# microsoft/Sora

Measured on AMD Instinct MI355X. Metric: IQ Msamples/s through 802.11a 54 Mbps RX PHY, higher is better.
Workload: dtype int16 IQ / u8 path metrics

## Files before the change

### sora_amd/build.py

```python
import os
import shutil
import subprocess
import sys
from concurrent.futures import ThreadPoolExecutor

HERE = os.path.dirname(os.path.abspath(__file__))
CSRC = os.path.join(HERE, "csrc")
OBJ = os.path.join(HERE, "lib", "obj")
LIB = os.path.join(HERE, "lib", "libsora_hip.so")
SOURCES = ["k_scan.hip", "k_rx.hip", "k_vit16.hip", "k_vitwin.hip", "k_stage.hip", "k_tx.hip", "k_tx11n.hip", "k_tx_ht40.hip", "k_tx11b.hip", "k_rx11b.hip", "k_11n.hip", "k_rx11n.hip",
    "k_ht40.hip", "k_deliver.hip", "sora_hip.cpp", "sora_shard.cpp"]
HEADERS = ["dev_arith.h", "dev_viterbi.h", "dev_vit16.h", "dev_winplan.h", "dev_vitwin.h", "dev_11n.h", "dev_ht40.h", "dev_pilot11a.h", "dev_sym11a.h", "rx_types.h", "kernels.h", "host_calls.h",
           "host_trellis.h", os.path.join("..", "..", "include", "sora_hip.h")]
FLAGS = ["--offload-arch=gfx950", "-O3", "-std=c++17", "-fPIC", "-fvisibility=hidden", "-x", "hip"]


def hipcc():
    for c in (os.environ.get("HIPCC"), shutil.which("hipcc"), "/opt/rocm/bin/hipcc"):
        if c and os.path.exists(c):
            return c
    raise RuntimeError("hipcc not found: libsora_hip.so cannot be built (there is no CPU fallback)")


def _newest_header():
    return max(os.path.getmtime(os.path.join(CSRC, h)) for h in HEADERS)


def _obj(src):
    return os.path.join(OBJ, os.path.splitext(src)[0] + ".o")


def _stale(src, hdr_t):
    o = _obj(src)
    return not os.path.exists(o) or os.path.getmtime(o) < max(os.path.getmtime(os.path.join(CSRC, src)), hdr_t)


def needs_build():
    if not os.path.exists(LIB):
        return True
    t = os.path.getmtime(LIB)
    return any(os.path.getmtime(os.path.join(CSRC, f)) > t for f in SOURCES + HEADERS)


INFO = os.path.join(HERE, "lib", "libsora_hip.buildinfo.json")


def sources_sha256():
    import hashlib
    h = hashlib.sha256()
    for f in sorted(SOURCES) + sorted(HEADERS):
        with open(os.path.join(CSRC, f), "rb") as fh:
            h.update(f.encode()); h.update(fh.read())
    return h.hexdigest()


def build_info():
    import json, socket, hashlib
    out = {"library": os.path.relpath(LIB, os.path.dirname(HERE)), "exists": os.path.exists(LIB)}
    if out["exists"]:
        with open(LIB, "rb") as fh:
            out["library_sha256"] = hashlib.sha256(fh.read()).hexdigest()
    try:
        with open(INFO) as fh:
            st = json.load(fh)
    except Exception:
        st = None
    now = sources_sha256()
    out["stamp"] = st
    out["sources_sha256_now"] = now
    out["built_from_this_tree"] = bool(st) and st.get("sources_sha256") == now and st.get("library_sha256") == out.get("library_sha256")
    out["built_on_this_host"] = bool(st) and st.get("host") == socket.gethostname()
    return out


def _write_info(ncompiled):
    import json, socket, hashlib, time
    try:
        ver = subprocess.run([hipcc(), "--version"], capture_output=True, text=True).stdout.splitlines()[0]
    except Exception:
        ver = None
    with open(LIB, "rb") as fh:
        lib_sha = hashlib.sha256(fh.read()).hexdigest()
    with open(INFO, "w") as fh:
        json.dump({"sources_sha256": sources_sha256(), "library_sha256": lib_sha, "host": socket.gethostname(), "built_at_unix": int(time.time()), "hipcc": ver,
                   "flags": FLAGS, "objects_compiled_in_this_build": ncompiled}, fh, indent=1)


def build_variant(name, defines):
    out_dir = os.path.join(HERE, "lib", "variants"); os.makedirs(out_dir, exist_ok=True)
    out = os.path.join(out_dir, name + ".so")
    if any(d.startswith(("SORA_DBG_", "SORA_SCAN_PROBE")) for d in defines) and "SORA_TOOLS" not in defines:
        defines = list(defines) + ["SORA_TOOLS"]
    cmd = [hipcc()] + FLAGS + ["-shared", "-w"] + ["-D" + d for d in defines] + [os.path.join(CSRC, f) for f in SOURCES] + ["-ldl", "-o", out]
    subprocess.check_call(cmd)
    return out

# ... 30 lines not shown
```

### sora_amd/csrc/k_rx.hip

```cpp
#include <hip/hip_runtime.h>
#include <utility>
#include "kernels.h"
#include "dev_sym11a.h"
#include "dev_viterbi.h"
#include "dev_winplan.h"
#include "dev_vitwin.h"

namespace sora {

struct FrameLds {
    uint32_t eq[4][4][64];
    uint8_t  soft[4][4][288];
    uint8_t  demap[1024];
    int4     trk[4][4];
    int      nsym_of[4];
    short    st0[4][4];
};
template <bool SHARED>
__device__ __forceinline__ void frame_symbols(const RxArgs& A, uint32_t j, FrameLds& lds, bool valid = true)
{
    uint32_t (&s_eq)[4][4][64] = lds.eq; uint8_t (&s_soft)[4][4][288] = lds.soft; const uint8_t* s_demap = lds.demap;
    const int w = threadIdx.x >> 6, lane = threadIdx.x & 63, g = lane >> 4, e = lane & 15;
    const Tables& T = A.T;
    const uint32_t f = valid ? A.joblist[j] : 0u;
// ... 784 lines not shown
        if (w < nwords) {
            const uint32_t sb = phase == 255 ? 0u : lds.seq4[(phase + 32u * w) % 127u];
            const uint32_t o = __builtin_amdgcn_alignbyte(hi[k], lo[k], 2u) ^ sb;
            s_buf[w] = o;
            mp32[w] = o;
            if (hp32) hp32[w] = o;
        }
    }
    __builtin_amdgcn_fence(__ATOMIC_RELEASE, "wavefront");
    __builtin_amdgcn_wave_barrier();
    __builtin_amdgcn_fence(__ATOMIC_ACQUIRE, "wavefront");
    const int n = L >= 4 ? (int)L - 4 : 0;
    uint32_t crc;
    if (n >= 4) {
        crc = crc32_wave(bytes, n, s_crc, s_z, lane);
    } else {
        crc = 0xFFFFFFFFu;
        for (int i = 0; i < n; i++) crc = (crc >> 8) ^ s_crc[(bytes[i] ^ crc) & 0xFF];
    }
    if (lane == 0) {
        uint32_t fcs = 0;
        if (L >= 4) fcs = (uint32_t)bytes[L - 4] | ((uint32_t)bytes[L - 3] << 8) | ((uint32_t)bytes[L - 2] << 16) | ((uint32_t)bytes[L - 1] << 24);
        r.crc32 = fcs;
        r.error_code = ((~crc) == fcs) ? E_FRAME_OK : E_CRC32_FAIL;
    }
}

__global__ void __launch_bounds__(256) k_finish(RxArgs A)
{
    __shared__ FinishLds L;
    finish_tables_to_lds(A, L);
    __syncthreads();
    const JobRef jr = locate_job(blockIdx.x * 4 + (threadIdx.x >> 6), A.njobs);
    if (!jr.ok) return;
    finish_frame(A, A.joblist[jr.list * A.nrows + jr.idx], L);
}

struct PipeFallbackGate {
    WinProofGate proof; const RxArgs* A; FrameLds* lds; bool gave_up;
    __device__ __forceinline__ bool operator()(uint32_t list, uint32_t fa, uint32_t fb, bool hasB) const
    {
        if (!gave_up) return proof(list, fa, fb, hasB);
        frame_symbols<false>(*A, list * A->nrows + fa, *lds);
        if (hasB) frame_symbols<false>(*A, list * A->nrows + fb, *lds);
        __builtin_amdgcn_fence(__ATOMIC_RELEASE, "agent"); __builtin_amdgcn_fence(__ATOMIC_ACQUIRE, "agent");
        return true;
    }
};
template <bool PIPE>
__device__ __forceinline__ void win_redo_finish_body(const VitJob* jobs, const uint32_t* hdr, uint32_t jstride, uint32_t target, uint32_t vstride,
                                                     const uint16_t* vecs, const uint8_t* soft, uint8_t* out, unsigned long long* stats, const RxArgs& A, uint32_t* host_note)
{
    __shared__ FinishLds L;
    finish_tables_to_lds(A, L);
    auto after = [&](uint32_t list, uint32_t fa, uint32_t fb, bool hasB) {
        finish_frame(A, A.joblist[list * A.nrows + fa], L);
        if (hasB) finish_frame(A, A.joblist[list * A.nrows + fb], L);
    };
    const WinProofGate proof{ jobs, hdr, jstride, target, vstride, vecs, stats };
    if constexpr (PIPE) {
        __shared__ FrameLds F;
        reinterpret_cast<uint32_t*>(F.demap)[threadIdx.x] = reinterpret_cast<const uint32_t*>(A.T.demap)[threadIdx.x];
        __syncthreads();
        const bool gave_up = __builtin_amdgcn_readfirstlane((int)A.pipe_flags[0]) != 0;
        if (gave_up && blockIdx.x == 0 && threadIdx.x == 0) {
            if (stats) atomicAdd(&stats[4u * kWinStatBanks], 1ull);
            if (host_note) __hip_atomic_store(host_note, 1u, __ATOMIC_RELAXED, __HIP_MEMORY_SCOPE_SYSTEM);
        }
        viterbi_kernel_body<256, 24, 3>(jobs, hdr, 0u, jstride, soft, out, PipeFallbackGate{ proof, &A, &F, gave_up }, after);
    } else {
        __syncthreads();
        viterbi_kernel_body<256, 24, 3>(jobs, hdr, 0u, jstride, soft, out, proof, after);
    }
}
__global__ void __launch_bounds__(256) k_win_redo_finish(const VitJob* jobs, const uint32_t* hdr, uint32_t jstride, uint32_t target, uint32_t vstride,
                                                         const uint16_t* vecs, const uint8_t* soft, uint8_t* out, unsigned long long* stats, RxArgs A)
{ win_redo_finish_body<false>(jobs, hdr, jstride, target, vstride, vecs, soft, out, stats, A, nullptr); }
__global__ void __launch_bounds__(256) k_win_redo_finish_pipe(const VitJob* jobs, const uint32_t* hdr, uint32_t jstride, uint32_t target, uint32_t vstride,
                                                              const uint16_t* vecs, const uint8_t* soft, uint8_t* out, unsigned long long* stats, RxArgs A, uint32_t* host_note)
{ win_redo_finish_body<true>(jobs, hdr, jstride, target, vstride, vecs, soft, out, stats, A, host_note); }

struct PackedRow { uint32_t capture_id, start_sample, end_sample, error_code, rate_kbps; uint16_t length, nsym; uint32_t crc32; int16_t cfo_est;
    uint16_t flags; uint32_t mpdu_offset; };
__global__ void __launch_bounds__(1024) k_pack(const FrameRow* frames, const uint32_t* nframes, const CapDesc* caps, uint32_t ncaps, uint32_t max_frames,
                                               PackedRow* rows, uint32_t* nrows_out)
{
    __shared__ uint32_t s_scan[1024];
    __shared__ uint32_t s_base;
    const uint32_t t = threadIdx.x;
    if (t == 0) s_base = 0;
    __syncthreads();
    for (uint32_t c0 = 0; c0 < ncaps; c0 += 1024) {
        const uint32_t c = c0 + t;
        const uint32_t found = c < ncaps ? nframes[c] : 0u;
        const uint32_t n = min(found, max_frames);
        s_scan[t] = n;
        __syncthreads();
        for (uint32_t o = 1; o < 1024; o <<= 1) {
            const uint32_t v = t >= o ? s_scan[t - o] : 0u;
            __syncthreads();
            s_scan[t] += v;
            __syncthreads();
        }
        const uint32_t first = s_base + s_scan[t] - n;
        for (uint32_t i = 0; i < n; i++) {
            const FrameRow& r = frames[(size_t)c * max_frames + i];
            PackedRow o;
            o.capture_id = caps[c].capture_id; o.start_sample = r.start_sample; o.end_sample = r.end_sample; o.error_code = r.error_code;
            o.rate_kbps = r.rate_kbps; o.length = r.length; o.nsym = r.nsym; o.crc32 = r.crc32; o.cfo_est = r.cfo_est;
            o.flags = (i + 1 == n && found > max_frames) ? 1u : 0u;
            o.mpdu_offset = r.slot0 * (uint32_t)kOutPerSlot;
            rows[first + i] = o;
        }
        __syncthreads();
        if (t == 1023) s_base += s_scan[1023];
        __syncthreads();
    }
    if (t == 0) *nrows_out = s_base;
}


__global__ void __launch_bounds__(256) k_soft_pack3(const uint8_t* soft8, const uint32_t* off8, const uint32_t* nsoft, const uint16_t* flen, const uint32_t* out_off,
                                                    int code_rate, uint8_t* packed, VitJob* jobs)
{
    const uint32_t j = blockIdx.x, mine = nsoft[j], at = (off8[j] + 1u) / 2u;
    const uint8_t* in = soft8 + off8[j];
    for (uint32_t g = threadIdx.x; g < (mine + 7u) / 8u; g += blockDim.x) {
        uint32_t v[8];
#pragma unroll
        for (int k = 0; k < 8; k++) v[k] = 8u * g + k < mine ? in[8u * g + k] & 7u : 0u;
        const uint32_t bits24 = soft3_pack8(v), left = mine - 8u * g;
        if (left >= 8u) soft3_store8(packed + at, g, bits24);
        else for (uint32_t b = 0; b < (3u * left + 7u) / 8u; b++) packed[at + 3u * g + b] = (uint8_t)(bits24 >> (8u * b));
    }
    if (threadIdx.x == 0) {
        VitJob J; J.soft_off = at; J.nsoft = mine; J.length = flen[j]; J.dec_off = 0; J.out_off = out_off[j];
        J.valid = 1; J.code_rate = (uint32_t)code_rate; J.soft_bits = 3;
        jobs[j] = J;
    }
}

__global__ void __launch_bounds__(256) k_soft_jobs8(const uint32_t* off8, const uint32_t* nsoft, const uint16_t* flen, const uint32_t* out_off, int code_rate,
                                                    uint32_t n, VitJob* jobs)
{
    const uint32_t j = blockIdx.x * blockDim.x + threadIdx.x;
    if (j >= n) return;
    VitJob J; J.soft_off = off8[j]; J.nsoft = nsoft[j]; J.length = flen[j]; J.dec_off = 0; J.out_off = out_off[j];
    J.valid = 1; J.code_rate = (uint32_t)code_rate; J.soft_bits = 8;
    jobs[j] = J;
}

}
```

### sora_amd/csrc/kernels.h

```cpp
#pragma once
#include <hip/hip_runtime.h>
#include <vector>
#include "dev_arith.h"
#include "rx_types.h"
#include "../../include/sora_hip.h"

#if !defined(SORA_TOOLS) && (defined(SORA_SCAN_PROBE) || defined(SORA_DBG_PIPE_TIMELINE) || defined(SORA_DBG_PIPE_LOSE_FLAGS))
#error "SORA_SCAN_PROBE / SORA_DBG_* switches need -DSORA_TOOLS (sora_amd.build.build_variant)"
#endif

namespace sora {

struct ScanArgs {
    const uint32_t* iq;
    const CapDesc*  caps;
    uint32_t        ncaps;
    uint32_t        str;
    uint32_t        keep_queue;
    uint32_t        thr;
    uint32_t        max_frames;
    Tables          T;
    FrameRow*       frames;
    FrameCtx*       fctx;
    uint32_t*       nframes;
    uint32_t*       njobs;
    uint32_t*       joblist;
    uint32_t        nrows;
    uint32_t*       slot_row;
    uint32_t*       cont;
    uint32_t*       consumed;
    uint32_t*       zero_a; uint32_t nzero_a;
    uint32_t*       zero_b; uint32_t nzero_b;
    uint32_t        own_slots;
};
constexpr int kContWords = 64;

struct RxArgs {
    const uint32_t* iq;
    const CapDesc*  caps;
    uint32_t        str;
    uint32_t        total_slots;
    uint32_t        nrows;
    Tables          T;
    FrameRow*       frames;
    const FrameCtx* fctx;
    uint8_t*        soft;
    uint8_t*        vout;
    uint8_t*        mpdu;
    VitJob*         jobs;
    const uint32_t* njobs;
    const uint32_t* joblist;
    const uint32_t* slot_row;
    uint32_t*       eq;
    TrackRec*       track;
    uint32_t*       pil;
    const uint32_t* pipe_flags;
    uint8_t*        mpdu_host;
};

struct PipeArgs {
    uint32_t  nfront, ntrack;
    uint32_t* flags;
    uint32_t  target, vstride;
    uint16_t* vecs;
    uint32_t  stamp_base;
    uint32_t  lanes64;
    uint32_t  wait_ticks;
};

__global__ void k_scan(ScanArgs A);
__global__ void k_frame(RxArgs A);
__global__ void k_sym_front(RxArgs A);
__global__ void k_track_lds(RxArgs A);
__global__ void k_sym_back(RxArgs A);
__global__ void k_pipe(RxArgs A, PipeArgs P);
__global__ void k_viterbi(const VitJob* jobs, const uint32_t* njobs3, uint32_t njobs_single, uint32_t stride, const uint8_t* soft, uint8_t* out);
__global__ void k_viterbi11n(const VitJob* jobs, const uint32_t* njobs3, uint32_t njobs_single, uint32_t stride, const uint8_t* soft, uint8_t* out);
__global__ void k_viterbi16(const VitJob* jobs, const uint32_t* njobs3, uint32_t njobs_single, uint32_t stride, const uint8_t* soft, uint8_t* out);
__global__ void k_viterbi16_11n(const VitJob* jobs, const uint32_t* njobs3, uint32_t njobs_single, uint32_t stride, const uint8_t* soft, uint8_t* out);
__global__ void k_viterbi16w(const VitJob* jobs, const uint32_t* hdr, uint32_t jstride, uint32_t target, uint32_t vstride, const uint8_t* soft, uint8_t* out, uint16_t* vecs);
__global__ void k_viterbi16w_11n(const VitJob* jobs, const uint32_t* hdr, uint32_t jstride, uint32_t target, uint32_t vstride, const uint8_t* soft, uint8_t* out, uint16_t* vecs);
__global__ void k_win_redo_11n(const VitJob* jobs, const uint32_t* hdr, uint32_t jstride, uint32_t target, uint32_t vstride, const uint16_t* vecs,
        const uint8_t* soft, uint8_t* out, unsigned long long* stats);
__global__ void k_win_redo(const VitJob* jobs, const uint32_t* hdr, uint32_t jstride, uint32_t target, uint32_t vstride, const uint16_t* vecs,
        const uint8_t* soft, uint8_t* out, unsigned long long* stats);
__global__ void k_win_redo_finish(const VitJob* jobs, const uint32_t* hdr, uint32_t jstride, uint32_t target, uint32_t vstride, const uint16_t* vecs,
        const uint8_t* soft, uint8_t* out, unsigned long long* stats,
                                  RxArgs A);
__global__ void k_win_redo_finish_pipe(const VitJob* jobs, const uint32_t* hdr, uint32_t jstride, uint32_t target, uint32_t vstride, const uint16_t* vecs,
        const uint8_t* soft, uint8_t* out, unsigned long long* stats, RxArgs A, uint32_t* host_note);
__global__ void k_finish(RxArgs A);
struct PackedRow;
__global__ void k_pack(const FrameRow* frames, const uint32_t* nframes, const CapDesc* caps, uint32_t ncaps, uint32_t max_frames, PackedRow* rows, uint32_t* nrows_out);
__global__ void k_fft64_batch(const uint32_t* in, uint32_t* out, uint32_t n, Tables T);
template <int NB> __global__ void k_demap_batch(const uint32_t* in, uint8_t* soft, uint32_t n, Tables T);
template <int NB> __global__ void k_deint_batch(const uint8_t* in, uint8_t* out, uint32_t n, Tables T);
__global__ void k_lts_batch(const uint32_t* in, uint32_t* ctx, uint32_t n, Tables T);
__global__ void k_symfront_batch(const uint32_t* in, const uint32_t* ctx, const uint32_t* ctx_index, uint32_t* eq, uint32_t n, Tables T);
template <bool PHASE> __global__ void k_ptrack_batch(const uint32_t* eq, const uint32_t* first, const uint32_t* nsym, uint32_t* state, uint32_t* out, uint32_t nframes, Tables T);
template <int KIND> __global__ void k_cmul64_batch(const uint32_t* in, const uint32_t* coef, uint32_t cstride, uint32_t coff, const uint32_t* cindex, uint32_t* out, uint32_t n);
__global__ void k_fft128_batch(const uint32_t* in, uint32_t* out, uint32_t n, Tables T);
struct TxArgs {
    const uint8_t*  mpdu;
    const uint32_t* off;
    const uint32_t* len;
    const uint32_t* rate;
    const uint8_t*  seed;
    int8_t*         out8;
    const uint64_t* out_off;
    const int8_t*   preamble;
    Tables          T;
};
__global__ void k_tx_preamble(int8_t* out8, int8_t* out44, Tables T);
template <bool UP44> __global__ void k_tx11a(TxArgs A);

struct Tx11nArgs {
    const uint8_t*  mpdu;
    const uint32_t* off;
    const uint32_t* len;
    const uint32_t* mcs;
    const uint8_t*  seed;
    uint32_t*       out0;
    uint32_t*       out1;
    const uint64_t* out_off;
    const uint32_t* preamble;
    Tables          T;
};
struct Tx11nPlan { int nb, cr, ndbps; uint32_t nstd, nbytes, nvalid, nsym; };
__host__ __device__ inline bool tx11n_plan(uint32_t len, uint32_t mcs, Tx11nPlan& P)
{
    if (len < 1 || len > 4092) return false;
    switch (mcs) {
    case 8:  P.nb = 1; P.cr = 0; P.ndbps = 52;  break;  case 9:  P.nb = 2; P.cr = 0; P.ndbps = 104; break;
    case 10: P.nb = 2; P.cr = 2; P.ndbps = 156; break;  case 11: P.nb = 4; P.cr = 0; P.ndbps = 208; break;
    case 12: P.nb = 4; P.cr = 2; P.ndbps = 312; break;  case 13: P.nb = 6; P.cr = 1; P.ndbps = 416; break;
    case 14: P.nb = 6; P.cr = 2; P.ndbps = 468; break;
    default: return false;
    }
    const uint32_t nd = (uint32_t)P.ndbps, gin = (uint32_t)P.cr + 1, gout = (uint32_t)P.cr + 2;
    P.nstd = ((len + 4) * 8 + 16 + 6 + nd - 1) / nd;
    P.nbytes = (P.nstd * nd + 7) / 8;
    const uint32_t ngroups = (P.nbytes + gin - 1) / gin;
    P.nvalid = 8 * gin * ngroups;
    P.nsym = (gout * ngroups + 13 * (uint32_t)P.nb - 1) / (13 * (uint32_t)P.nb);
    return true;
}
constexpr uint32_t kTx11nPreamble = 1120;
__global__ void k_tx11n(Tx11nArgs A);

struct TxHt40Args {
    const uint8_t*  mpdu;
    const uint32_t* off;
    const uint32_t* len;
    const uint32_t* mcs;
    const uint8_t*  seed;
    uint32_t*       out0;
    uint32_t*       out1;
    const uint64_t* out_off;
    const uint32_t* preamble;
    Tables          T;
};
struct TxHt40Plan { int nb, cr, ndbps; uint32_t nsym; };
__host__ __device__ inline bool tx_ht40_plan(uint32_t len, uint32_t mcs, TxHt40Plan& P)
{
    if (len < 1 || len > 3996) return false;
    switch (mcs) {
    case 8:  P.nb = 1; P.cr = 0; P.ndbps = 54;  break;  case 9:  P.nb = 2; P.cr = 0; P.ndbps = 108; break;
    case 10: P.nb = 2; P.cr = 2; P.ndbps = 162; break;  case 11: P.nb = 4; P.cr = 0; P.ndbps = 216; break;
    case 12: P.nb = 4; P.cr = 2; P.ndbps = 324; break;  case 13: P.nb = 6; P.cr = 1; P.ndbps = 432; break;
    case 14: P.nb = 6; P.cr = 2; P.ndbps = 486; break;
    default: return false;
    }
    P.nsym = (16u + 8u * (len + 4u) + 6u + (uint32_t)P.ndbps - 1u) / (uint32_t)P.ndbps;
    return true;
}
// ... 99 lines not shown
```

### sora_amd/csrc/sora_hip.cpp

```cpp
#include <hip/hip_runtime.h>
#include <cmath>
#include <cstdio>
#include <cstdlib>
#include <cstring>
#include <algorithm>
#include <atomic>
#include <chrono>
#include <mutex>
#include <string>
#include <vector>
#include "../../include/sora_hip.h"
#include "kernels.h"
#include "host_trellis.h"

using namespace sora;

static thread_local std::string g_last_error;
hipError_t sora_internal_stream_create(hipStream_t* out, int index)
{
    int least = 0, greatest = 0;
    (void)hipDeviceGetStreamPriorityRange(&least, &greatest);
    const int level = index % 3, prio = level == 0 ? 0 : level == 1 ? greatest : least;
    if (least != greatest) return hipStreamCreateWithPriority(out, hipStreamNonBlocking, prio);
    return hipStreamCreateWithFlags(out, hipStreamNonBlocking);
}

static int fail(int code, const char* what, hipError_t e = hipSuccess)
{
    char buf[256];
    if (e != hipSuccess) snprintf(buf, sizeof(buf), "%s: %s", what, hipGetErrorString(e));
    else snprintf(buf, sizeof(buf), "%s", what);
    g_last_error = buf;
    return code;
}

struct HostTables {
    std::vector<int16_t> usin, ucos, uatan2;
    std::vector<uint8_t> demap;
    std::vector<uint32_t> tw64, tw16, sts, crc, tw128, tw32, tw8, rot;
    std::vector<uint16_t> deint;
    std::vector<uint8_t> scr, scr_seq, scr_phase;
    std::vector<uint32_t> crcz;
    std::vector<uint32_t> trk;
};

static inline uint32_t pk(int re, int im) { return ((uint32_t)re & 0xFFFFu) | ((uint32_t)im << 16); }

namespace hostfft {
struct c { int re, im; };
static inline int w16(int v) { return (int)(short)v; }
static inline int sat(int v) { return v > 32767 ? 32767 : (v < -32768 ? -32768 : v); }
static inline c mk(int r, int i) { c x; x.re = r; x.im = i; return x; }
static inline c sra(c a, int n) { return mk(a.re >> n, a.im >> n); }
static inline c adds(c a, c b) { return mk(sat(a.re + b.re), sat(a.im + b.im)); }
static inline c subs(c a, c b) { return mk(sat(a.re - b.re), sat(a.im - b.im)); }
static inline c cnot(c a) { return mk(~a.re, ~a.im); }
static inline c conj_mul_shift15(c a, c b)
{
    int v0 = (int)((unsigned)(a.re * b.re) + (unsigned)(a.im * b.im));
    int v1 = (int)((unsigned)(a.im * b.re) + (unsigned)(w16(-a.re) * b.im));
    return mk(w16(v0 >> 15), w16(v1 >> 15));
}
static void stage(c* x, int n, const std::vector<c>* tw)
{
    const int q = n / 4;
    for (int e = 0; e < q; e++) {
        c a = sra(x[e], 2), b = sra(x[e + q], 2), cc = sra(x[e + 2 * q], 2), d = sra(x[e + 3 * q], 2);
        c ac = adds(a, cc), bd = adds(b, d), a_c = subs(a, cc), b_d = subs(b, d);
        c jb = mk(~b_d.im, b_d.re);
        x[e] = adds(ac, bd);
        x[e + q] = conj_mul_shift15(subs(ac, bd), tw[1][e]);
        x[e + 2 * q] = conj_mul_shift15(adds(a_c, jb), tw[0][e]);
        x[e + 3 * q] = conj_mul_shift15(subs(a_c, jb), tw[2][e]);
    }
}
static void t4(c* x)
{
    c s0 = sra(x[0], 2), s1 = sra(x[1], 2), s2 = sra(x[2], 2), s3 = sra(x[3], 2);
    c A0 = adds(s0, s2), A1 = adds(s1, s3), B0 = adds(cnot(s2), s0), B1 = adds(cnot(s3), s1);
    c B1r = mk(~B1.im, B1.re);
    x[0] = adds(A0, A1); x[1] = adds(cnot(A1), A0); x[2] = adds(B0, B1r); x[3] = adds(cnot(B1r), B0);
}
}

static void build_tables(HostTables& H)
{
    const double GEN_PI = 3.141593;
    H.usin.resize(65536); H.ucos.resize(65536); H.uatan2.resize(65536);
    for (int i = 0; i < 65536; i++) {
        double x = (double)i * GEN_PI / 32768.0;
        H.usin[i] = (int16_t)std::floor(32767.0 * std::sin(x) + 0.5);
        H.ucos[i] = (int16_t)std::floor(32767.0 * std::cos(x) + 0.5);
    }
    H.rot.resize(65536);
    for (int i = 0; i < 65536; i++) H.rot[i] = pk(H.ucos[i], -(int)H.usin[i]);
    for (int yi = 0; yi < 256; yi++)
        for (int xi = 0; xi < 256; xi++) {
            int t = (int)(std::atan2((double)(int8_t)yi, (double)(int8_t)xi) * 32768.0 / GEN_PI);
            H.uatan2[yi * 256 + xi] = (int16_t)(t > 32767 ? 32767 : t);
        }
    struct St { int at, val; };
    static const St bpsk[] = {{-128,0},{-30,1},{-17,2},{-8,3},{0,4},{9,5},{18,6},{31,7}};
    static const St q16[]  = {{-128,0},{-70,1},{-67,2},{-65,3},{-63,4},{-61,5},{-58,6},{-55,7},{56,6},{59,5},{62,4},{64,3},{66,2},{68,1},{71,0}};
    static const St q64a[] = {{-128,0},{-68,1},{-65,2},{-63,3},{-61,4},{-60,5},{-58,6},{-55,7},{56,6},{59,5},{61,4},{62,3},{64,2},{66,1},{69,0}};
    static const St q64b[] = {{-128,0},{-98,1},{-96,2},{-94,3},{-92,4},{-90,5},{-89,6},{-86,7},{-37,6},{-34,5},{-32,4},{-30,3},{-29,2},{-27,1},{-24,0},
// ... 629 lines not shown
                               rx->win.stride, (const uint16_t*)rx->win.d_vecs, (const uint8_t*)rx->d_soft, rx->d_vout, rx->win.d_stats, R);
        else if (RX_ONLY(rx, 8u)) hipLaunchKernelGGL(k_finish, dim3((nrows + 3) / 4), dim3(256), 0, st, R);
#ifdef SORA_TOOLS
        for (unsigned x = 0; x < rx->extra; x++) hipLaunchKernelGGL(k_clear16, dim3(1), dim3(256), 0, st, reinterpret_cast<uint4*>(rx->d_njobs), 0u);
#endif
        mark();
        return SORA_OK;
    };

    const bool repeat = rx->last_valid && !caps_changed && rx->last_iq == (const void*)d_iq && rx->last_bound == (const void*)rx->bound_mpdu;
    rx->last_bound = rx->bound_mpdu;
    if (!repeat && rx->graph_exec) {
        (void)hipGraphExecDestroy(rx->graph_exec); rx->graph_exec = nullptr;
        (void)hipGraphDestroy(rx->graph); rx->graph = nullptr;
    }
    rx->last_iq = d_iq; rx->last_valid = true;
    bool launched = false;
    if (rx->use_graph && !prof && repeat && !rx->ordered) {
        if (!rx->graph_exec) {
            if (hipStreamBeginCapture(st, hipStreamCaptureModeThreadLocal) == hipSuccess) {
                const int rc = enqueue(true);
                hipGraph_t g = nullptr;
                const hipError_t e2 = hipStreamEndCapture(st, &g);
                if (rc == SORA_OK && e2 == hipSuccess && g && hipGraphInstantiate(&rx->graph_exec, g, nullptr, nullptr, 0) == hipSuccess) rx->graph = g;
                else { if (g) (void)hipGraphDestroy(g); rx->graph_exec = nullptr; rx->use_graph = false; (void)hipGetLastError(); }
            } else { rx->use_graph = false; (void)hipGetLastError(); }
        }
        if (rx->graph_exec) { HIPCHK(hipGraphLaunch(rx->graph_exec, st)); launched = true; }
    }
    if (!launched) { const int rc = enqueue(false); if (rc) return rc; }
    HIPCHK(hipGetLastError());
    rx->ev_valid = prof;
    rx->have_results = true;
    return SORA_OK;
}

static int pipe_process(RxPipe* rx, const sora_complex16* h_iq, size_t total_samples, const sora_capture_desc* caps, size_t ncaps)
{
    if (!rx || !h_iq) return fail(SORA_ERR_INVALID_PARAM, "sora_rx_process: null argument");
    if (total_samples > rx->cfg.max_total_samples) return fail(SORA_ERR_CAPACITY, "more samples than sora_rx_cfg.max_total_samples");
    HIPCHK(hipSetDevice(rx->cfg.device));
    if (rx->iq_own_samples < total_samples) {
        if (rx->d_iq_own) (void)hipFree(rx->d_iq_own);
        rx->d_iq_own = nullptr; rx->iq_own_samples = 0;
        HIPCHK(hipMalloc((void**)&rx->d_iq_own, sizeof(sora_complex16) * (total_samples + 64)));
        rx->iq_own_samples = total_samples;
    }
    HIPCHK(hipMemcpyAsync(rx->d_iq_own, h_iq, sizeof(sora_complex16) * total_samples, hipMemcpyHostToDevice, rx->stream));
    return pipe_process_dev(rx, rx->d_iq_own, caps, ncaps, total_samples);
}

static int pipe_process_dump(RxPipe* rx, const void* h_dump, size_t dump_bytes, unsigned flags, const sora_capture_desc* caps, size_t ncaps)
{
    if (!rx || !h_dump || dump_bytes == 0) return fail(SORA_ERR_INVALID_PARAM, "sora_rx_process_dump: null argument");
    if ((flags & ~15u) || (dump_bytes & 3)) return fail(SORA_ERR_INVALID_PARAM,
            "sora_rx_process_dump: unknown ingest flag, or a dump that is not a whole number of 4-byte samples");
    const size_t n = sora_hip_ingest_count(dump_bytes, flags);
    if (n > rx->cfg.max_total_samples) return fail(SORA_ERR_CAPACITY, "sora_rx_process_dump: the dump holds more samples than sora_rx_cfg.max_total_samples");
    HIPCHK(hipSetDevice(rx->cfg.device));
    if (rx->dump_cap < dump_bytes || rx->iq_own_samples < n) HIPCHK(hipStreamSynchronize(rx->stream));
    if (rx->dump_cap < dump_bytes) {
        if (rx->d_dump) (void)hipFree(rx->d_dump);
        rx->d_dump = nullptr; rx->dump_cap = 0;
        HIPCHK(hipMalloc((void**)&rx->d_dump, dump_bytes + 256));
        rx->dump_cap = dump_bytes;
    }
    if (rx->iq_own_samples < n) {
        if (rx->d_iq_own) (void)hipFree(rx->d_iq_own);
        rx->d_iq_own = nullptr; rx->iq_own_samples = 0;
        HIPCHK(hipMalloc((void**)&rx->d_iq_own, sizeof(sora_complex16) * (n + 64)));
        rx->iq_own_samples = n;
    }
    HIPCHK(hipMemcpyAsync(rx->d_dump, h_dump, dump_bytes, hipMemcpyHostToDevice, rx->stream));
    size_t got = 0;
    const int rc = sora_hip_ingest(rx->d_dump, dump_bytes, flags, rx->d_iq_own, rx->iq_own_samples, &got, (void*)rx->stream);
    if (rc != SORA_OK) return rc;
    return pipe_process_dev(rx, rx->d_iq_own, caps, ncaps, got);
}

static int pipe_pack(RxPipe* rx)
{
    static_assert(sizeof(sora_frame_result) == 36, "sora_frame_result layout");
    if (rx->ncaps == 0) HIPCHK(hipMemsetAsync(rx->d_nrows, 0, 4, rx->stream));
    else hipLaunchKernelGGL(k_pack, dim3(1), dim3(1024), 0, rx->stream, (const FrameRow*)rx->d_frames, (const uint32_t*)rx->d_nframes,
                            (const CapDesc*)rx->d_caps, rx->ncaps, rx->cfg.max_frames_per_capture, reinterpret_cast<PackedRow*>(rx->d_rows), rx->d_nrows);
    HIPCHK(hipGetLastError());
    return SORA_OK;
}

static int pipe_results(RxPipe* rx, sora_frame_result* out, size_t max_out, size_t* nout, uint8_t* h_mpdu, size_t mpdu_cap)
{
    if (!rx || !nout) return fail(SORA_ERR_INVALID_PARAM, "sora_rx_results: null argument");
    *nout = 0;
    if (!rx->have_results) return fail(SORA_ERR_FAILED, "no process call to report");
    if (rx->ncaps == 0) return SORA_OK;
    HIPCHK(hipSetDevice(rx->cfg.device));
    { const int rc = pipe_pack(rx); if (rc) return rc; }
    uint32_t nrows = 0;
    HIPCHK(hipMemcpyAsync(&nrows, rx->d_nrows, 4, hipMemcpyDeviceToHost, rx->stream));
    HIPCHK(hipStreamSynchronize(rx->stream));
    std::vector<sora_frame_result> rows(nrows);
    if (nrows) HIPCHK(hipMemcpy(rows.data(), rx->d_rows, sizeof(sora_frame_result) * (size_t)nrows, hipMemcpyDeviceToHost));
    std::vector<uint8_t> mp;
    if (h_mpdu && nrows) { mp.resize((size_t)kOutPerSlot * rx->total_slots); HIPCHK(hipMemcpy(mp.data(), rx->d_mpdu, mp.size(), hipMemcpyDeviceToHost)); }
    size_t n = 0, moff = 0; int rc = SORA_OK;
    for (uint32_t i = 0; i < nrows; i++) {
        if (n >= max_out) { rc = SORA_ERR_CAPACITY; break; }
        sora_frame_result& o = out[n++];
        o = rows[i];
        const size_t src = o.mpdu_offset;
        o.mpdu_offset = (uint32_t)moff;
        if (h_mpdu && (o.error_code == E_FRAME_OK || o.error_code == E_CRC32_FAIL)) {
            if (moff + o.length > mpdu_cap) { rc = SORA_ERR_CAPACITY; continue; }
            memcpy(h_mpdu + moff, mp.data() + src, o.length);
            moff += o.length;
        }
    }
    *nout = n;
    if (rc != SORA_OK) return fail(rc, "sora_rx_results: output buffer too small");
    return SORA_OK;
}

static int pipe_set_profiling(RxPipe* rx, int enable)
{
    if (!rx) return SORA_ERR_INVALID_PARAM;
    HIPCHK(hipSetDevice(rx->cfg.device));
    if (enable && !rx->ev[0]) for (auto& e : rx->ev) HIPCHK(hipEventCreate(&e));
    rx->profiling = enable != 0; rx->ev_valid = false;
    for (auto& t : rx->t_sum) t = 0.0;
    rx->t_calls = 0;
    return SORA_OK;
}

const char* sora_rx_kernel_name(size_t i) { return i < kNumTimed ? kKernelNames[i] : ""; }
const char* sora_rx_kernel_name_fused(size_t i) { return i < kNumTimed ? kKernelNamesFused[i] : ""; }

static int pipe_results_dev(RxPipe* rx, const sora_frame_result** d_rows, const uint32_t** d_nrows, const uint8_t** d_mpdu)
{
    if (!rx) return fail(SORA_ERR_INVALID_PARAM, "sora_rx_results_dev: null handle");
    if (!rx->have_results) return fail(SORA_ERR_FAILED, "no process call to report");
    HIPCHK(hipSetDevice(rx->cfg.device));
    { const int rc = pipe_pack(rx); if (rc) return rc; }
    if (d_rows) *d_rows = rx->d_rows;
    if (d_nrows) *d_nrows = rx->d_nrows;
    if (d_mpdu) *d_mpdu = rx->d_mpdu;
    return SORA_OK;
}

static int pipe_deliver_async(RxPipe* rx, sora_frame_result* h_rows, size_t max_rows, uint32_t* h_nrows, uint8_t* h_mpdu, size_t mpdu_bytes)
{
    if (!rx || !h_rows || !h_nrows) return fail(SORA_ERR_INVALID_PARAM, "sora_rx_deliver_async: null argument");
    if (!rx->have_results) return fail(SORA_ERR_FAILED, "no process call to report");
    const size_t need = (size_t)kOutPerSlot * rx->total_slots;
    if (h_mpdu && mpdu_bytes < need) return fail(SORA_ERR_CAPACITY, "sora_rx_deliver_async: h_mpdu is smaller than sora_rx_mpdu_bytes()");
    HIPCHK(hipSetDevice(rx->cfg.device));
    { const int rc = pipe_pack(rx); if (rc) return rc; }
    const size_t nr = std::min<size_t>(max_rows, (size_t)rx->ncaps * rx->cfg.max_frames_per_capture);
    HIPCHK(hipMemcpyAsync(h_nrows, rx->d_nrows, 4, hipMemcpyDeviceToHost, rx->stream));
    if (nr) HIPCHK(hipMemcpyAsync(h_rows, rx->d_rows, sizeof(sora_frame_result) * nr, hipMemcpyDeviceToHost, rx->stream));
    if (h_mpdu && need && h_mpdu != rx->bound_mpdu) HIPCHK(hipMemcpyAsync(h_mpdu, rx->d_mpdu, need, hipMemcpyDeviceToHost, rx->stream));
    HIPCHK(call_mark_delivered(*rx));
    return SORA_OK;
}

}

constexpr long long kAutoLanes16Captures = 32768;
// ... 961 lines not shown
```

Measured before the change: 53720.

## Parallelize result packing across blocks with wave scans; rebalance stream priority levels

Rewrites k_pack from a single 1024-thread block with an LDS Hillis-Steele scan into up to 16 blocks of 256 threads. Each block first sums the preceding captures' frame counts and then runs wave-shuffle prefix scans with a small LDS hop between waves, which drops the many per-step barriers. Separately, stream priority levels are now assigned by a queue-capacity-aware round robin instead of index%3. The extra blocks each redundantly re-read all earlier counts, and the stream change alters the priority mix for every pipeline stream.

```diff
diff --git a/sora_amd/build.py b/sora_amd/build.py
--- a/sora_amd/build.py
+++ b/sora_amd/build.py
@@ -11,7 +11,7 @@
 SOURCES = ["k_scan.hip", "k_rx.hip", "k_vit16.hip", "k_vitwin.hip", "k_stage.hip", "k_tx.hip", "k_tx11n.hip", "k_tx_ht40.hip", "k_tx11b.hip", "k_rx11b.hip", "k_11n.hip", "k_rx11n.hip",
     "k_ht40.hip", "k_deliver.hip", "sora_hip.cpp", "sora_shard.cpp"]
 HEADERS = ["dev_arith.h", "dev_viterbi.h", "dev_vit16.h", "dev_winplan.h", "dev_vitwin.h", "dev_11n.h", "dev_ht40.h", "dev_pilot11a.h", "dev_sym11a.h", "rx_types.h", "kernels.h", "host_calls.h",
-           "host_trellis.h", os.path.join("..", "..", "include", "sora_hip.h")]
+           "host_trellis.h", "host_streams.h", os.path.join("..", "..", "include", "sora_hip.h")]
 FLAGS = ["--offload-arch=gfx950", "-O3", "-std=c++17", "-fPIC", "-fvisibility=hidden", "-x", "hip"]
 
 
diff --git a/sora_amd/csrc/host_streams.h b/sora_amd/csrc/host_streams.h
--- /dev/null
+++ b/sora_amd/csrc/host_streams.h
@@ -0,0 +1,23 @@
+#pragma once
+
+namespace sora {
+
+constexpr int kStreamLevels = 3;
+constexpr int kFreeQueues[kStreamLevels] = { 3, 4, 4 };
+constexpr int kOwnQueueStreams = kFreeQueues[0] + kFreeQueues[1] + kFreeQueues[2];
+
+constexpr int stream_level(int index)
+{
+    int used[kStreamLevels] = { 0, 0, 0 }, level = kStreamLevels - 1;
+    for (int i = 0; i <= index; i++) {
+        const int round = i < kOwnQueueStreams ? 0 : 1 + (i - kOwnQueueStreams) / kStreamLevels;
+        for (int k = 0; k < kStreamLevels; k++) {
+            level = (level + 1) % kStreamLevels;
+            if (used[level] < kFreeQueues[level] + round) break;
+        }
+        used[level]++;
+    }
+    return level;
+}
+
+}
diff --git a/sora_amd/csrc/k_rx.hip b/sora_amd/csrc/k_rx.hip
--- a/sora_amd/csrc/k_rx.hip
+++ b/sora_amd/csrc/k_rx.hip
@@ -890,27 +890,32 @@
 
 struct PackedRow { uint32_t capture_id, start_sample, end_sample, error_code, rate_kbps; uint16_t length, nsym; uint32_t crc32; int16_t cfo_est;
     uint16_t flags; uint32_t mpdu_offset; };
-__global__ void __launch_bounds__(1024) k_pack(const FrameRow* frames, const uint32_t* nframes, const CapDesc* caps, uint32_t ncaps, uint32_t max_frames,
-                                               PackedRow* rows, uint32_t* nrows_out)
-{
-    __shared__ uint32_t s_scan[1024];
-    __shared__ uint32_t s_base;
-    const uint32_t t = threadIdx.x;
-    if (t == 0) s_base = 0;
+__global__ void __launch_bounds__(kPackThreads) k_pack(const FrameRow* frames, const uint32_t* nframes, const CapDesc* caps, uint32_t ncaps, uint32_t max_frames,
+                                                        PackedRow* rows, uint32_t* nrows_out)
+{
+    static_assert(kPackThreads == 256, "four waves: the LDS hop below");
+    __shared__ uint32_t s_wave[2][4];
+    __shared__ uint32_t s_before[4];
+    const uint32_t t = threadIdx.x, lane = t & 63u, w = t >> 6;
+    const uint32_t tiles = (ncaps + kPackThreads - 1u) / kPackThreads, per = (tiles + gridDim.x - 1u) / gridDim.x;
+    const uint32_t c_begin = min(blockIdx.x * per * kPackThreads, ncaps), c_end = min(c_begin + per * kPackThreads, ncaps);
+    uint32_t before = 0;
+    for (uint32_t c = t; c < c_begin; c += kPackThreads) before += min(nframes[c], max_frames);
+    for (int d = 32; d > 0; d >>= 1) before += (uint32_t)__shfl_xor((int)before, d);
+    if (lane == 0) s_before[w] = before;
     __syncthreads();
-    for (uint32_t c0 = 0; c0 < ncaps; c0 += 1024) {
+    uint32_t base = s_before[0] + s_before[1] + s_before[2] + s_before[3];
+    uint32_t set = 0;
+    for (uint32_t c0 = c_begin; c0 < c_end; c0 += kPackThreads, set ^= 1u) {
         const uint32_t c = c0 + t;
         const uint32_t found = c < ncaps ? nframes[c] : 0u;
         const uint32_t n = min(found, max_frames);
-        s_scan[t] = n;
+        uint32_t incl = n;
+        for (int d = 1; d < 64; d <<= 1) { const uint32_t v = (uint32_t)__shfl_up((int)incl, d); if (lane >= (uint32_t)d) incl += v; }
+        if (lane == 63u) s_wave[set][w] = incl;
         __syncthreads();
-        for (uint32_t o = 1; o < 1024; o <<= 1) {
-            const uint32_t v = t >= o ? s_scan[t - o] : 0u;
-            __syncthreads();
-            s_scan[t] += v;
-            __syncthreads();
-        }
-        const uint32_t first = s_base + s_scan[t] - n;
+        const uint32_t w0 = s_wave[set][0], w1 = s_wave[set][1], w2 = s_wave[set][2], w3 = s_wave[set][3];
+        const uint32_t first = base + (w > 0 ? w0 : 0u) + (w > 1 ? w1 : 0u) + (w > 2 ? w2 : 0u) + incl - n;
         for (uint32_t i = 0; i < n; i++) {
             const FrameRow& r = frames[(size_t)c * max_frames + i];
             PackedRow o;
@@ -920,11 +925,9 @@
             o.mpdu_offset = r.slot0 * (uint32_t)kOutPerSlot;
             rows[first + i] = o;
         }
-        __syncthreads();
-        if (t == 1023) s_base += s_scan[1023];
-        __syncthreads();
-    }
-    if (t == 0) *nrows_out = s_base;
+        base += w0 + w1 + w2 + w3;
+    }
+    if (blockIdx.x + 1u == gridDim.x && t == 0) *nrows_out = base;
 }
 
 
diff --git a/sora_amd/csrc/kernels.h b/sora_amd/csrc/kernels.h
--- a/sora_amd/csrc/kernels.h
+++ b/sora_amd/csrc/kernels.h
@@ -91,6 +91,16 @@
         const uint8_t* soft, uint8_t* out, unsigned long long* stats, RxArgs A, uint32_t* host_note);
 __global__ void k_finish(RxArgs A);
 struct PackedRow;
+constexpr uint32_t kPackThreads = 256;
+#ifndef SORA_PACK_MAX_GROUPS
+#define SORA_PACK_MAX_GROUPS 16
+#endif
+constexpr uint32_t kPackMaxGroups = SORA_PACK_MAX_GROUPS;
+inline uint32_t pack_groups(uint32_t ncaps)
+{
+    const uint32_t tiles = (ncaps + kPackThreads - 1u) / kPackThreads, per = (tiles + kPackMaxGroups - 1u) / kPackMaxGroups;
+    return (tiles + per - 1u) / per;
+}
 __global__ void k_pack(const FrameRow* frames, const uint32_t* nframes, const CapDesc* caps, uint32_t ncaps, uint32_t max_frames, PackedRow* rows, uint32_t* nrows_out);
 __global__ void k_fft64_batch(const uint32_t* in, uint32_t* out, uint32_t n, Tables T);
 template <int NB> __global__ void k_demap_batch(const uint32_t* in, uint8_t* soft, uint32_t n, Tables T);
diff --git a/sora_amd/csrc/sora_hip.cpp b/sora_amd/csrc/sora_hip.cpp
--- a/sora_amd/csrc/sora_hip.cpp
+++ b/sora_amd/csrc/sora_hip.cpp
@@ -12,6 +12,7 @@
 #include "../../include/sora_hip.h"
 #include "kernels.h"
 #include "host_trellis.h"
+#include "host_streams.h"
 
 using namespace sora;
 
@@ -20,7 +21,7 @@
 {
     int least = 0, greatest = 0;
     (void)hipDeviceGetStreamPriorityRange(&least, &greatest);
-    const int level = index % 3, prio = level == 0 ? 0 : level == 1 ? greatest : least;
+    const int level = sora::stream_level(index), prio = level == 0 ? 0 : level == 1 ? greatest : least;
     if (least != greatest) return hipStreamCreateWithPriority(out, hipStreamNonBlocking, prio);
     return hipStreamCreateWithFlags(out, hipStreamNonBlocking);
 }
@@ -816,7 +817,7 @@
 {
     static_assert(sizeof(sora_frame_result) == 36, "sora_frame_result layout");
     if (rx->ncaps == 0) HIPCHK(hipMemsetAsync(rx->d_nrows, 0, 4, rx->stream));
-    else hipLaunchKernelGGL(k_pack, dim3(1), dim3(1024), 0, rx->stream, (const FrameRow*)rx->d_frames, (const uint32_t*)rx->d_nframes,
+    else hipLaunchKernelGGL(k_pack, dim3(pack_groups(rx->ncaps)), dim3(kPackThreads), 0, rx->stream, (const FrameRow*)rx->d_frames, (const uint32_t*)rx->d_nframes,
                             (const CapDesc*)rx->d_caps, rx->ncaps, rx->cfg.max_frames_per_capture, reinterpret_cast<PackedRow*>(rx->d_rows), rx->d_nrows);
     HIPCHK(hipGetLastError());
     return SORA_OK;
```

Result: faster. 54410 (median of 5 runs) (+1.3%).
